# open-genome/dna

Measured on AMD Instinct MI355X. Metric: MLM sequences/sec, DNABERT-2-117M seq_len=512, at 1/2/4/8 MI355X, higher is better.
Workload: dtype bf16

## Files before the change

### dna_amd/_native.py

```python
import ctypes
import os
import re

import torch

_HERE = os.path.dirname(os.path.abspath(__file__))
LIB_PATH = os.environ.get("DNA_AMD_LIB", os.path.join(_HERE, "lib", "libdna_amd.so"))
HEADER = os.path.join(os.path.dirname(_HERE), "include", "dna_amd.h")

F32, BF16, F16 = 0, 1, 2
ACT_NONE, ACT_GELU = 0, 1

_vp, _i, _u64, _f, _sz = ctypes.c_void_p, ctypes.c_int, ctypes.c_uint64, ctypes.c_float, ctypes.c_size_t
_i64 = ctypes.c_int64

_SIGS = {
    "dna_abi_version": (_i, []),
    "dna_last_error": (ctypes.c_char_p, []),
    "dna_attn_fwd": (_i, [_vp, _vp, _vp, _i, _i, _i, _i, _i, _f, _vp, _vp, _vp]),
    "dna_attn_bwd": (_i, [_vp, _vp, _vp, _vp, _vp, _vp, _i, _i, _i, _i, _i, _f, _vp, _vp, _vp]),
    "dna_attn_bwd_ex": (_i, [_vp, _vp, _vp, _vp, _vp, _vp, _i, _i, _i, _i, _i, _f, _vp, _vp, _vp, _vp]),
    "dna_attn_dbias_part_rows": (_i, [_i, _i]),
    "dna_flash_lse_rows": (_i, [_i]),
    "dna_flash_fwd": (_i, [_vp, _i, _vp, _i, _i, _i64, _i64, _i64, _i, _i, _i, _i, _i, _f, _vp, _vp, _vp]),
    "dna_flash_bwd": (_i, [_vp, _i, _vp, _i, _i, _i64, _i64, _i64, _vp, _vp, _vp, _i, _i, _i, _i, _i,
                           _f, _vp, _vp, _vp]),
    "dna_colsum_f32": (_i, [_vp, _i, _i, _vp, _i, _vp]),
    "dna_colsum_bf16_workspace": (_sz, [_i, _i]),
    "dna_colsum_bf16": (_i, [_vp, _i, _i, _vp, _i, _vp, _sz, _vp]),
    "dna_flip_rows": (_i, [_vp, _i, _i, _sz, _vp, _vp]),
    "dna_causal_conv1d_fwd": (_i, [_vp, _sz, _i, _vp, _vp, _i, _i, _i, _i, _i, _vp, _vp]),
    "dna_causal_conv1d_part_rows": (_sz, [_i, _i]),
    "dna_causal_conv1d_bwd": (_i, [_vp, _sz, _i, _vp, _vp, _vp, _i, _i, _i, _i, _i, _vp, _sz, _vp, _vp]),
    "dna_hyena_shortconv_fwd": (_i, [_vp, _i, _vp, _vp, _i, _i, _i, _i, _i, _vp, _vp, _vp]),
    "dna_hyena_shortconv_part_elems": (_sz, [_i, _i, _i, _i, _i]),
    "dna_hyena_shortconv_bwd": (_i, [_vp, _i, _vp, _vp, _i, _i, _i, _i, _i, _vp, _vp, _vp, _vp, _vp]),
    "dna_hyena_gate_out_fwd": (_i, [_vp, _vp, _i, _i, _i, _i, _sz, _vp, _vp]),
    "dna_hyena_gate_out_bwd": (_i, [_vp, _vp, _vp, _i, _i, _i, _i, _sz, _vp, _vp, _vp]),
    "dna_hyena_modulate_t_fwd": (_i, [_vp, _i, _vp, _vp, _f, _i, _i, _i, _vp, _vp]),
    "dna_hyena_modulate_t_bwd": (_i, [_vp, _vp, _vp, _f, _i, _i, _i, _vp, _i, _vp]),
    "dna_hyena_filter_part_elems": (_i, [_i, _i, _i, _i]),
    "dna_hyena_filter_part_stride": (_i, [_i, _i, _i]),
    "dna_hyena_filter_fwd": (_i, [_vp, _vp, _vp, _vp, _vp, _i, _vp, _vp, _vp, _vp, _f, _i, _i, _i, _i,
                                  _vp, _vp]),
    "dna_hyena_filter_bwd": (_i, [_vp, _vp, _vp, _vp, _vp, _i, _vp, _vp, _vp, _vp, _f, _i, _i, _i, _i,
                                  _vp, _vp, _vp, _vp]),
    "dna_hyena_filter_finish": (_i, [_vp, _i, _i, _i, _vp, _vp]),
    "dna_ln_fwd": (_i, [_vp, _i, _vp, _i, _f, _u64, _u64, _vp, _vp, _vp, _i, _i, _f, _vp, _vp,
                        _vp, _vp, _vp]),
    "dna_ln_bwd_workspace": (_sz, [_i, _i]),
    "dna_ln_bwd": (_i, [_vp, _vp, _vp, _i, _vp, _i, _f, _u64, _u64, _vp, _vp, _vp, _vp, _i, _i,
                        _vp, _vp, _vp, _vp, _vp, _vp, _sz, _vp]),
    "dna_ln_bwd_from_y": (_i, [_vp, _vp, _vp, _i, _f, _u64, _u64, _vp, _vp, _vp, _i, _i, _vp,
                               _vp, _vp, _vp, _vp, _vp, _sz, _vp]),
# ... 124 lines not shown
```

### dna_amd/csrc/attention.hip

```cpp
#include <stdlib.h>

#include <algorithm>
#include <type_traits>

#include "common.h"

namespace dna {
namespace attn {

constexpr int D = 64;
constexpr int BQ = 128;
constexpr int BK = 64;
constexpr float LOG2E = 1.4426950408889634f;
constexpr float LN2 = 0.6931471805599453f;
constexpr float PAD_BIAS = -10000.0f;

typedef __attribute__((address_space(3))) bf16x4 lds_bf16x4;
typedef __attribute__((ext_vector_type(4))) short s16x4;

__device__ __forceinline__ int swz_key(int r) {
  const int k = (r >> 1) & 7;
  return ((k & 1) << 2) | (k & 2) | ((k >> 2) & 1);
}
__device__ __forceinline__ int swz(int r, int c) {
// ... 1264 lines not shown
__device__ __forceinline__ float sum32(float x) {
  x += dppf<0xB1>(x);
  x += dppf<0x4E>(x);
  x += dppf<0x141>(x);
  x += dppf<0x140>(x);
  return x + __shfl_xor(x, 16, 64);
}

__device__ __forceinline__ void mfma_acc(f32x16& acc, const bf16x8& a, const bf16x8& b) {
  asm volatile("s_nop 1\n\tv_mfma_f32_32x32x16_bf16 %0, %1, %2, %0" : "+a"(acc) : "v"(a), "v"(b));
}
__device__ __forceinline__ void acc_fence(f32x16& x, f32x16& y) {
  asm volatile("s_nop 7\n\ts_nop 7\n\ts_nop 7" : "+a"(x), "+a"(y));
}

template <int KB>
constexpr size_t bwd3_red_off() {
  constexpr size_t a = (size_t)128 * KB * D * 2 + 4 * 32 * D * 2 + (size_t)128 * KB * 32 * 2 + 2 * 4 * 32 * 4;
  return a > 65536 ? a : 65536;
}
constexpr int CS_LD = 36;
template <int KB>
constexpr bool bwd3_stage_alias() { return (size_t)4 * 32 * D * 2 + (size_t)128 * KB * 32 * 2 >= 4 * 64 * CS_LD * 4; }
template <int KB>
constexpr size_t bwd3_lds() {
  return bwd3_red_off<KB>() + 2 * 1024 * 4 + (size_t)128 * KB * 2 * 4 +
         (bwd3_stage_alias<KB>() ? 0 : 4 * 64 * CS_LD * 4);
}

#ifndef DNA_BWD3_STAMP
#define DNA_BWD3_STAMP 0
#endif
#if DNA_BWD3_STAMP
__device__ unsigned long long g_bwd3_stamps[4][16][6];
#define BWD3_STAMP(t, k)                                                              \
  do {                                                                                \
    const unsigned long long ts_ = __builtin_amdgcn_s_memtime();                     \
    if (blockIdx.x == 0 && lane == 0 && (t) < 16) g_bwd3_stamps[wave][(t)][(k)] = ts_; \
  } while (0)
#else
#define BWD3_STAMP(t, k) do {} while (0)
#endif
template <int KB, int V>
__global__ __launch_bounds__(256, 1) void bwd3_bf16_kernel(
    const bf16* __restrict__ qkv, const bf16* __restrict__ out, const bf16* __restrict__ dout,
    const float* __restrict__ lse, const uint8_t* __restrict__ key_valid,
    const float* __restrict__ slopes, int H, float c, float scale, bf16* __restrict__ dqkv,
    float* __restrict__ dbias_part) {
  constexpr bool DB = V & 1;
  constexpr bool DBL = DB, DBE = DB;
  constexpr bool PIPE_SB = (V & 2) != 0;
  constexpr int S = 128 * KB;
  constexpr int KPW = 32 * KB;
  constexpr int NS = S / 32;
  constexpr int KS2 = S / 32;
  extern __shared__ __attribute__((aligned(16))) char smem[];
  bf16* Kimg = reinterpret_cast<bf16*>(smem);
  bf16* Qimg = Kimg + S * D;
  bf16* Oimg = Qimg + 2 * 32 * D;
  bf16* dST = Oimg + 2 * 32 * D;
  float* rc = reinterpret_cast<float*>(dST + S * 32);
  float* red = reinterpret_cast<float*>(smem + bwd3_red_off<KB>());

  const int bh = blockIdx.x, h = bh % H, b = bh / H;
  const int tid = threadIdx.x, lane = tid & 63;
  const int wave = __builtin_amdgcn_readfirstlane(tid >> 6);
  const int kl = lane & 31, hh = lane >> 5;
  const int g16 = lane >> 4, i16 = lane & 15;
  const int ld = 3 * H * D;
  const bf16* base = qkv + (size_t)b * S * ld;
  const size_t obase = (size_t)b * S * (H * D) + h * D;
  const float slope2 = slopes[h] * LOG2E;
  const float invc = 1.f / c;
  const float sl_t = slope2 * invc;
  const float* lse_bh = lse + ((size_t)b * H + h) * S;

  {
    constexpr int NCH = S * 8 / 256;
    bf16x8 kt[NCH];
#pragma unroll
    for (int i = 0; i < NCH; ++i) {
      const int cc = tid + 256 * i;
      kt[i] = *reinterpret_cast<const bf16x8*>(base + (size_t)(cc >> 3) * ld + H * D + h * D + (cc & 7) * 8);
    }
#pragma unroll
    for (int i = 0; i < NCH; ++i) {
      const int cc = tid + 256 * i;
      *reinterpret_cast<bf16x8*>(Kimg + swz(cc >> 3, (cc & 7) * 8)) = kt[i];
    }
  }
  bf16x8 vf[KB][4];
  unsigned padm = 0;
#pragma unroll
  for (int kb = 0; kb < KB; ++kb) {
    const int kj = wave * KPW + 32 * kb + kl;
#pragma unroll
    for (int s = 0; s < 4; ++s)
      vf[kb][s] = *reinterpret_cast<const bf16x8*>(base + (size_t)kj * ld + 2 * H * D + h * D + 16 * s + 8 * hh);
    if (key_valid && !key_valid[(size_t)b * S + kj]) padm |= 1u << kb;
  }

  struct SRegs { bf16x8 q, o, d; float l; };
  auto load_slice = [&](int t, SRegs& x, int tid_t) {
    const int sr = tid_t >> 3, sc = tid_t & 7;
    const int q = 32 * t + sr;
    x.q = *reinterpret_cast<const bf16x8*>(base + (size_t)q * ld + h * D + sc * 8);
    x.o = *reinterpret_cast<const bf16x8*>(out + obase + (size_t)q * (H * D) + sc * 8);
    x.d = *reinterpret_cast<const bf16x8*>(dout + obase + (size_t)q * (H * D) + sc * 8);
// ... 9 lines not shown
    dl += dppf<0xB1>(dl);
    dl += dppf<0x4E>(dl);
    dl += dppf<0x141>(dl);
    if (sc == 0) {
      const float l2 = x.l * LOG2E, sq = slope2 * (float)(32 * t + sr);
      float* R = rc + buf * 128 + sr;
      R[0] = (-l2 - sq) * invc;
      R[32] = (-l2 + sq) * invc;
      R[64] = -l2 * invc;
      R[96] = -dl;
    }
  };

  f32x16 dk[KB][2], dv[KB][2];
  float* sigl = red + 2 * 1024;
  if (DBL)
    for (int i = tid; i < 2 * S; i += 256) sigl[i] = 0.f;
#pragma unroll
  for (int kb = 0; kb < KB; ++kb) {
#pragma unroll
    for (int i = 0; i < 16; ++i) { dk[kb][0][i] = dk[kb][1][i] = dv[kb][0][i] = dv[kb][1][i] = 0.f; }
  }
  const int dth = wave & 1, kh2 = wave >> 1;
  const bf16* Kw = Kimg + wave * KPW * D;
  bf16* dSTw = dST + wave * KPW * 32;
  const bf16* Kh = Kimg + kh2 * (S / 2) * D;
  const bf16* dSTh = dST + kh2 * (S / 2) * 32;
  {
    SRegs x;
    load_slice(0, x, tid);
    store_slice(0, 0, x, tid);
  }
  __syncthreads();

  for (int t = 0; t < NS; ++t) {
    BWD3_STAMP(t, 0);
    const int buf = t & 1;
    int tid_t = tid;
    asm volatile("" : "+v"(tid_t));
    const int kl_t = tid_t & 31;
    unsigned padm_t = padm;
    asm volatile("" : "+v"(padm_t));
    SRegs nx;
    const bf16* Q = Qimg + buf * 32 * D;
    const bf16* O = Oimg + buf * 32 * D;
    const float* RC = rc + buf * 128;
    const int qb = 32 * t;
    bf16x8 pbp[2], sbp[2];
    const int tq = 4 * (g16 >> 1) + (i16 >> 2);
    auto tr_pair = [&](const bf16* img, int j) {
      const int qrow = 16 * (j >> 1) + tq;
      const int dcol = 32 * (j & 1) + 16 * (g16 & 1) + 4 * (i16 & 3);
      return cat(tr_read(img + swz(qrow, dcol)), tr_read(img + swz(qrow + 8, dcol)));
    };
    bf16x8 qfr[4], ofr[4];
#pragma unroll
    for (int s = 0; s < 4; ++s) {
      qfr[s] = *reinterpret_cast<const bf16x8*>(Q + swz(kl, 16 * s + 8 * hh));
      ofr[s] = *reinterpret_cast<const bf16x8*>(O + swz(kl, 16 * s + 8 * hh));
    }
#pragma unroll
    for (int kb = 0; kb <= KB; ++kb) {
      __builtin_amdgcn_sched_barrier(0);
      if (kb == KB && t + 1 < NS) load_slice(t + 1, nx, tid_t);
      const int kbase = wave * KPW + 32 * kb;
      const bool after = qb > kbase, before = qb < kbase;
// ... 98 lines not shown
      };
#pragma unroll
      for (int ks = 0; ks < PF; ++ks) rd(ks, ra[ks], rb[ks]);
#pragma unroll
      for (int ks = 0; ks < KS2; ++ks) {
        dq = mfma(ra[ks % PF], rb[ks % PF], dq);
        if (ks + PF < KS2) rd(ks + PF, ra[ks % PF], rb[ks % PF]);
      }
    }
    float* rw = red + dth * 1024;
#pragma unroll
    for (int g2 = 0; g2 < 2; ++g2) {
      const int g = 2 * (1 - kh2) + g2;
      *reinterpret_cast<f32x4*>(rw + g * 256 + lane * 4) = f32x4{dq[4 * g], dq[4 * g + 1], dq[4 * g + 2], dq[4 * g + 3]};
    }
    BWD3_STAMP(t, 3);
    if (t + 1 < NS) store_slice(buf ^ 1, t + 1, nx, tid_t);
    __syncthreads();
    BWD3_STAMP(t, 4);
    {
      bf16* row = dqkv + ((size_t)b * S + qb + kl) * ld + h * D + 32 * dth;
#pragma unroll
      for (int g2 = 0; g2 < 2; ++g2) {
        const int g = 2 * kh2 + g2;
        const f32x4 v = *reinterpret_cast<const f32x4*>(rw + g * 256 + lane * 4);
        bf16x4 o;
#pragma unroll
        for (int e = 0; e < 4; ++e) o[e] = (bf16)((dq[4 * g + e] + v[e]) * scale);
        *reinterpret_cast<bf16x4*>(row + 8 * g + 4 * hh) = o;
      }
    }
    BWD3_STAMP(t, 5);
  }

#pragma unroll
  for (int kb = 0; kb < KB; ++kb)
#pragma unroll
    for (int dt = 0; dt < 2; ++dt) acc_fence(dk[kb][dt], dv[kb][dt]);
#pragma unroll
  for (int kb = 0; kb < KB; ++kb) {
    bf16* row = dqkv + ((size_t)b * S + wave * KPW + 32 * kb + kl) * ld + h * D;
#pragma unroll
    for (int dt = 0; dt < 2; ++dt)
#pragma unroll
      for (int g = 0; g < 4; ++g) {
        bf16x4 vk, vv;
#pragma unroll
        for (int e = 0; e < 4; ++e) {
          vk[e] = (bf16)(dk[kb][dt][4 * g + e] * scale);
          vv[e] = (bf16)dv[kb][dt][4 * g + e];
        }
        *reinterpret_cast<bf16x4*>(row + H * D + 32 * dt + 8 * g + 4 * hh) = vk;
        *reinterpret_cast<bf16x4*>(row + 2 * H * D + 32 * dt + 8 * g + 4 * hh) = vv;
      }
  }
  if (DBE) {
#pragma unroll
    for (int kb = 0; kb < KB; ++kb)
#pragma unroll
      for (int dt = 0; dt < 2; ++dt) asm volatile("" : "+a"(dk[kb][dt]), "+a"(dv[kb][dt]));
    __syncthreads();
    int lane_e = lane;
    asm volatile("" : "+v"(lane_e));
    const int kl_e = lane_e & 31, hh_e = lane_e >> 5;
    float* cs = red;
    float* st = (bwd3_stage_alias<KB>() ? reinterpret_cast<float*>(Qimg)
                                        : red + 2 * 1024 + 2 * S) + wave * 64 * CS_LD;
    auto rowsum = [&](float* dst) {
      f32x4 a = *reinterpret_cast<const f32x4*>(st + lane_e * CS_LD);
#pragma unroll
      for (int k = 4; k < 32; k += 4) {
        const f32x4 v = *reinterpret_cast<const f32x4*>(st + lane_e * CS_LD + k);
        a[0] += v[0]; a[1] += v[1]; a[2] += v[2]; a[3] += v[3];
      }
      *dst = (a[0] + a[1]) + (a[2] + a[3]);
    };
    {
      float sgm[KB];
#pragma unroll
      for (int kb = 0; kb < KB; ++kb) {
        const int key = wave * KPW + 32 * kb + kl_e;
        sgm[kb] = sigl[key] + sigl[S + key];
      }
#pragma unroll
      for (int cc = 0; cc < 4; ++cc) {
        float a8[8] = {0.f, 0.f, 0.f, 0.f, 0.f, 0.f, 0.f, 0.f};
#pragma unroll
        for (int kb = 0; kb < KB; ++kb) {
          const int r = wave * KPW + 32 * kb + kl_e;
          const bf16x8 v = *reinterpret_cast<const bf16x8*>(Kimg + r * D + (((4 * hh_e + cc) ^ swz_key(r)) << 3));
#pragma unroll
          for (int e = 0; e < 8; ++e) a8[e] = fmaf((float)v[e], sgm[kb], a8[e]);
        }
#pragma unroll
        for (int e = 0; e < 8; ++e) st[(32 * hh_e + 8 * cc + e) * CS_LD + kl_e] = a8[e] * scale;
      }
      rowsum(cs + (wave * 3) * 64 + lane_e);
    }
#pragma unroll
    for (int ts = 0; ts < 2; ++ts) {
#pragma unroll
      for (int dt = 0; dt < 2; ++dt)
#pragma unroll
        for (int r = 0; r < 16; ++r) {
          float sum = 0.f;
#pragma unroll
          for (int kb = 0; kb < KB; ++kb) sum += ts == 0 ? dk[kb][dt][r] : dv[kb][dt][r];
          st[(32 * dt + aoff(r) + 4 * hh_e) * CS_LD + kl_e] = ts == 0 ? sum * scale : sum;
        }
      rowsum(cs + (wave * 3 + 1 + ts) * 64 + lane_e);
    }
    __syncthreads();
    for (int i = tid; i < KB * 192; i += 256) {
      const int j = i / 192, ts = (i >> 6) % 3, d = i & 63;
      float sum = 0.f;
#pragma unroll
      for (int w = 0; w < 4 / KB; ++w) sum += cs[((j * 4 / KB + w) * 3 + ts) * 64 + d];
      dbias_part[((size_t)b * KB + j) * ld + ts * H * D + h * D + d] = sum;
    }
  }
}

constexpr int F32_TILE = 64;

__device__ __forceinline__ float bias_nat(float slope, int i, int j, const uint8_t* kv, size_t off) {
  float bb = -slope * fabsf((float)(i - j));
  if (kv && !kv[off + j]) bb += PAD_BIAS;
  return bb;
}

__global__ __launch_bounds__(64) void fwd_f32_kernel(const float* __restrict__ qkv,
                                                      const uint8_t* __restrict__ kv,
                                                      const float* __restrict__ slopes, int S,
                                                      int H, float scale, float* __restrict__ out,
                                                      float* __restrict__ lse) {
  __shared__ float Kt[F32_TILE][D + 1], Vt[F32_TILE][D + 1];
  const int h = blockIdx.y, b = blockIdx.z, t = threadIdx.x;
  const int qi = blockIdx.x * F32_TILE + t;
  const int ld = 3 * H * D;
  const float* base = qkv + (size_t)b * S * ld;
  const float slope = slopes[h];
  float q[D], o[D];
  const int qr = min(qi, S - 1);
  for (int d = 0; d < D; ++d) { q[d] = base[(size_t)qr * ld + h * D + d]; o[d] = 0.f; }
  float m = -INFINITY, l = 0.f;
  for (int k0 = 0; k0 < S; k0 += F32_TILE) {
    __syncthreads();
    for (int idx = t; idx < F32_TILE * D; idx += 64) {
      int r = idx / D, d = idx % D, j = min(k0 + r, S - 1);
      Kt[r][d] = base[(size_t)j * ld + H * D + h * D + d];
      Vt[r][d] = base[(size_t)j * ld + 2 * H * D + h * D + d];
    }
    __syncthreads();
// ... 188 lines not shown
  }
  DNA_LAUNCH_CHECK("dna_attn_fwd");
  return DNA_OK;
}

template <int KB>
static void launch_bwd3(const void* qkv, const void* out, const void* dout, const float* lse,
                        const uint8_t* key_valid, const float* slopes, int batch, int heads, float c,
                        float scale, void* dqkv, float* dbias_part, hipStream_t s) {
  static const bool attr = [] {
    const void* ks[] = {(const void*)bwd3_bf16_kernel<KB, 0>, (const void*)bwd3_bf16_kernel<KB, 1>,
                        (const void*)bwd3_bf16_kernel<KB, 2>, (const void*)bwd3_bf16_kernel<KB, 3>};
    for (const void* k : ks)
      (void)hipFuncSetAttribute(k, hipFuncAttributeMaxDynamicSharedMemorySize, (int)bwd3_lds<KB>());
    return true;
  }();
  (void)attr;
  static const bool sb = getenv("DNA_ATTN_BWD3_SB") && atoi(getenv("DNA_ATTN_BWD3_SB")) == 1;
  const dim3 grid(batch * heads);
  const size_t lds = bwd3_lds<KB>();
  auto args = [&](auto kern, float* part) {
    hipLaunchKernelGGL(kern, grid, dim3(256), lds, s, (const bf16*)qkv, (const bf16*)out,
                       (const bf16*)dout, lse, key_valid, slopes, heads, c, scale, (bf16*)dqkv, part);
  };
  if (!dbias_part) {
    if (sb) args(bwd3_bf16_kernel<KB, 2>, nullptr);
    else args(bwd3_bf16_kernel<KB, 0>, nullptr);
  } else {
    if (sb) args(bwd3_bf16_kernel<KB, 3>, dbias_part);
    else args(bwd3_bf16_kernel<KB, 1>, dbias_part);
  }
}

extern "C" int dna_attn_bwd_ex(const void* qkv, const void* out, const void* dout,
                               const float* lse, const uint8_t* key_valid, const float* slopes,
                               int batch, int seqlen, int heads, int head_dim, int dtype,
                               float softmax_scale, void* dqkv, float* delta_ws, float* dbias_part,
                               void* stream) {
  int st = check_common(qkv, slopes, batch, seqlen, heads, head_dim, dtype, "dna_attn_bwd");
  if (st) return st;
  DNA_CHECK_ARG(out && dout && lse && dqkv && delta_ws, "dna_attn_bwd: null pointer");
  hipStream_t s = as_stream(stream);
  const int rows = batch * seqlen;
  const int nd = (rows * heads + 255) / 256;
  static const int bwd_ver = getenv("DNA_ATTN_BWD") ? atoi(getenv("DNA_ATTN_BWD")) : 3;
  const bool bwd_v1 = bwd_ver == 1;
  if (dtype == DNA_BF16 && bwd_ver == 3 && (seqlen == 128 || seqlen == 256 || seqlen == 512)) {
    const float c = softmax_scale * LOG2E;
    if (seqlen == 512)
      launch_bwd3<4>(qkv, out, dout, lse, key_valid, slopes, batch, heads, c, softmax_scale, dqkv, dbias_part, s);
    else if (seqlen == 256)
      launch_bwd3<2>(qkv, out, dout, lse, key_valid, slopes, batch, heads, c, softmax_scale, dqkv, dbias_part, s);
    else
      launch_bwd3<1>(qkv, out, dout, lse, key_valid, slopes, batch, heads, c, softmax_scale, dqkv, dbias_part, s);
  } else if (dtype == DNA_BF16 && !bwd_v1) {
    static const int nw_env = getenv("DNA_ATTN_BWD_NW") ? atoi(getenv("DNA_ATTN_BWD_NW")) : 8;
    const bool w8 = nw_env == 8 && seqlen % 256 == 0;
    const size_t red = (w8 ? 8 : 4) * 32 * 64 * sizeof(float);
    const size_t dq_lds = std::max(FWD_LDS, dbias_part ? red : (size_t)0);
    const size_t kv_lds = std::max(DKDV2_LDS, dbias_part ? red : (size_t)0);
    if (w8) {
      hipLaunchKernelGGL((dq2_bf16_kernel<8>), dim3((seqlen / 256) * heads * batch), dim3(512),
                         dq_lds, s, (const bf16*)qkv, (const bf16*)out, (const bf16*)dout, lse,
                         delta_ws, key_valid, slopes, seqlen, heads, softmax_scale * LOG2E,
                         softmax_scale, (bf16*)dqkv, dbias_part);
      hipLaunchKernelGGL((dkdv2_bf16_kernel<8>), dim3((seqlen / 256) * heads * batch), dim3(512),
                         kv_lds, s, (const bf16*)qkv, (const bf16*)dout, lse, delta_ws, key_valid,
                         slopes, seqlen, heads, softmax_scale * LOG2E, softmax_scale, (bf16*)dqkv,
                         dbias_part);
    } else {
      hipLaunchKernelGGL((dq2_bf16_kernel<4>), dim3(((seqlen + BQ - 1) / BQ) * heads * batch),
                         dim3(256), dq_lds, s, (const bf16*)qkv, (const bf16*)out,
                         (const bf16*)dout, lse, delta_ws, key_valid, slopes, seqlen, heads,
                         softmax_scale * LOG2E, softmax_scale, (bf16*)dqkv, dbias_part);
      hipLaunchKernelGGL((dkdv2_bf16_kernel<4>), dim3(((seqlen + BKW - 1) / BKW) * heads * batch),
                         dim3(256), kv_lds, s, (const bf16*)qkv, (const bf16*)dout, lse, delta_ws,
                         key_valid, slopes, seqlen, heads, softmax_scale * LOG2E, softmax_scale,
                         (bf16*)dqkv, dbias_part);
    }
  } else if (dtype == DNA_BF16) {
    hipLaunchKernelGGL(dq_bf16_kernel, dim3(((seqlen + BQ - 1) / BQ) * heads * batch), dim3(256),
                       FWD_LDS, s, (const bf16*)qkv, (const bf16*)out, (const bf16*)dout, lse,
                       delta_ws, key_valid, slopes, seqlen, heads, softmax_scale * LOG2E,
                       softmax_scale, (bf16*)dqkv, dbias_part);
    hipLaunchKernelGGL(dkdv_bf16_kernel, dim3(((seqlen + BKW - 1) / BKW) * heads * batch), dim3(256),
                       DKDV_LDS, s, (const bf16*)qkv, (const bf16*)dout, lse, delta_ws, key_valid,
                       slopes, seqlen, heads, softmax_scale * LOG2E, softmax_scale, (bf16*)dqkv,
                       dbias_part);
  } else {
    DNA_CHECK_ARG(!dbias_part, "dna_attn_bwd_ex: fused bias-gradient partials need the bf16 path");
    hipLaunchKernelGGL(delta_kernel<float>, dim3(nd), dim3(256), 0, s, (const float*)out,
                       (const float*)dout, rows, heads, seqlen, delta_ws);
    dim3 grid((seqlen + F32_TILE - 1) / F32_TILE, heads, batch);
    hipLaunchKernelGGL(dq_f32_kernel, grid, dim3(64), 0, s, (const float*)qkv, (const float*)dout,
                       lse, delta_ws, key_valid, slopes, seqlen, heads, softmax_scale,
                       (float*)dqkv);
    hipLaunchKernelGGL(dkdv_f32_kernel, grid, dim3(64), 0, s, (const float*)qkv,
                       (const float*)dout, lse, delta_ws, key_valid, slopes, seqlen, heads,
                       softmax_scale, (float*)dqkv);
  }
  DNA_LAUNCH_CHECK("dna_attn_bwd");
  return DNA_OK;
}

extern "C" int dna_attn_bwd(const void* qkv, const void* out, const void* dout, const float* lse,
                            const uint8_t* key_valid, const float* slopes, int batch, int seqlen,
                            int heads, int head_dim, int dtype, float softmax_scale, void* dqkv,
                            float* delta_ws, void* stream) {
  return dna_attn_bwd_ex(qkv, out, dout, lse, key_valid, slopes, batch, seqlen, heads, head_dim,
                         dtype, softmax_scale, dqkv, delta_ws, nullptr, stream);
}

#if DNA_BWD3_STAMP
extern "C" int dna_attn_debug_stamps(unsigned long long* out) {
  return hipMemcpyFromSymbol(out, HIP_SYMBOL(g_bwd3_stamps), sizeof(g_bwd3_stamps)) == hipSuccess ? 0 : 1;
}
#endif

extern "C" int dna_attn_dbias_part_rows(int batch, int seqlen) {
  return batch * ((seqlen + BQ - 1) / BQ);
}
```

### include/dna_amd.h

```cpp
#ifndef DNA_AMD_H
#define DNA_AMD_H

#include <stddef.h>
#include <stdint.h>

#ifdef __cplusplus
extern "C" {
#endif

#define DNA_AMD_ABI_VERSION 1

enum dna_status {
  DNA_OK = 0,
  DNA_ERR_INVALID = 1,
  DNA_ERR_HIP = 2,
  DNA_ERR_UNSUPPORTED = 3,
  DNA_ERR_IO = 4,
  DNA_ERR_NOMEM = 5
};

enum dna_dtype { DNA_F32 = 0, DNA_BF16 = 1, DNA_F16 = 2 };
enum dna_act { DNA_ACT_NONE = 0, DNA_ACT_GELU = 1 };

int dna_abi_version(void);
const char* dna_last_error(void);

int dna_attn_fwd(const void* qkv, const uint8_t* key_valid, const float* slopes, int batch,
                 int seqlen, int heads, int head_dim, int dtype, float softmax_scale, void* out,
                 float* lse, void* stream);

int dna_flash_lse_rows(int seqlen);
int dna_flash_fwd(const void* qkv, int dtype, const void* bias, int bias_dtype, int bias_type,
                  long long bias_sb, long long bias_sh, long long bias_sq, int batch, int seqlen,
                  int heads, int head_dim, int causal, float softmax_scale, void* out, float* lse,
                  void* stream);
int dna_flash_bwd(const void* qkv, int dtype, const void* bias, int bias_dtype, int bias_type,
                  long long bias_sb, long long bias_sh, long long bias_sq, const void* out,
                  const void* dout, const float* lse, int batch, int seqlen, int heads,
                  int head_dim, int causal, float softmax_scale, float* delta, void* dqkv,
                  void* stream);

int dna_attn_bwd(const void* qkv, const void* out, const void* dout, const float* lse,
                 const uint8_t* key_valid, const float* slopes, int batch, int seqlen, int heads,
                 int head_dim, int dtype, float softmax_scale, void* dqkv, float* delta_ws,
                 void* stream);
int dna_attn_bwd_ex(const void* qkv, const void* out, const void* dout, const float* lse,
                    const uint8_t* key_valid, const float* slopes, int batch, int seqlen, int heads,
                    int head_dim, int dtype, float softmax_scale, void* dqkv, float* delta_ws,
                    float* dbias_part, void* stream);
int dna_attn_dbias_part_rows(int batch, int seqlen);

int dna_ln_fwd(const void* x, int x_dtype, const float* bias, int act, float p_drop,
               uint64_t seed, uint64_t offset, const float* residual, const float* gamma,
               const float* beta, int rows, int cols, float eps, float* y, void* y_bf16,
               float* mean, float* rstd, void* stream);

size_t dna_ln_bwd_workspace(int rows, int cols);
int dna_ln_bwd(const float* dy, const void* dy_bf16, const void* x, int x_dtype,
               const float* bias, int act, float p_drop, uint64_t seed, uint64_t offset,
               const float* residual, const float* gamma, const float* mean, const float* rstd,
               int rows, int cols, float* dresidual, void* dx, float* dgamma, float* dbeta,
               float* dbias, void* workspace, size_t workspace_bytes, void* stream);
int dna_ln_bwd_from_y(const float* dy, const void* dy_bf16, const float* y, int x_dtype,
                      float p_drop, uint64_t seed, uint64_t offset, const float* gamma,
                      const float* beta, const float* rstd, int rows, int cols, float* dresidual,
                      void* dx, float* dgamma, float* dbeta, float* dbias, void* workspace,
                      size_t workspace_bytes, void* stream);
int dna_ln_bwd_from_y_acc(const float* dy, const void* dy_bf16, const float* y, int x_dtype,
                          float p_drop, uint64_t seed, uint64_t offset, const float* gamma,
                          const float* beta, const float* rstd, int rows, int cols,
                          float* dresidual, void* dx, float* dgamma, float* dbeta, float* dbias,
                          void* workspace, size_t workspace_bytes, void* stream);

int dna_add_ln_fwd(const void* x, int x_dtype, const float* residual, const float* gamma,
                   const float* beta, int rows, int cols, float eps, int rms, float* sum, float* y,
                   void* y_bf16, float* mean, float* rstd, void* stream);
int dna_add_ln_bwd(const float* dy, const void* dy_bf16, const float* dsum, const void* x,
                   int x_dtype, const float* residual, const float* gamma, const float* mean,
                   const float* rstd, int rows, int cols, int rms, float* dresidual, void* dx,
                   float* dgamma, float* dbeta, void* workspace, size_t workspace_bytes,
                   void* stream);

// ... 198 lines not shown
```

Measured before the change: 2425.

## Add 8-wave fused attention backward kernel and default to it at seq 512

Adds a new 512-thread attention backward kernel in which each of eight waves owns 32*KB keys, so a 512-token head is handled with KB=2 instead of the old 4-wave KB=4 layout. It uses raw LDS addressing with ds_read_tr transpose loads, a cross-wave dQ reduction through LDS, and stages dK/dV stores through the dead Q/O images. It becomes the default for seqlen 512, and a new dna_attn_bwd_var entry point selects 4 or 8 waves explicitly. The aim is more waves per CU and fewer accumulator registers per wave, traded against extra LDS reduction traffic and more barrier synchronisation.

```diff
diff --git a/dna_amd/_native.py b/dna_amd/_native.py
--- a/dna_amd/_native.py
+++ b/dna_amd/_native.py
@@ -20,6 +20,7 @@
     "dna_attn_fwd": (_i, [_vp, _vp, _vp, _i, _i, _i, _i, _i, _f, _vp, _vp, _vp]),
     "dna_attn_bwd": (_i, [_vp, _vp, _vp, _vp, _vp, _vp, _i, _i, _i, _i, _i, _f, _vp, _vp, _vp]),
     "dna_attn_bwd_ex": (_i, [_vp, _vp, _vp, _vp, _vp, _vp, _i, _i, _i, _i, _i, _f, _vp, _vp, _vp, _vp]),
+    "dna_attn_bwd_var": (_i, [_vp, _vp, _vp, _vp, _vp, _vp, _i, _i, _i, _i, _i, _f, _vp, _vp, _vp, _i, _vp]),
     "dna_attn_dbias_part_rows": (_i, [_i, _i]),
     "dna_flash_lse_rows": (_i, [_i]),
     "dna_flash_fwd": (_i, [_vp, _i, _vp, _i, _i, _i64, _i64, _i64, _i, _i, _i, _i, _i, _f, _vp, _vp, _vp]),
diff --git a/dna_amd/csrc/attention.hip b/dna_amd/csrc/attention.hip
--- a/dna_amd/csrc/attention.hip
+++ b/dna_amd/csrc/attention.hip
@@ -1320,11 +1320,11 @@
 #define DNA_BWD3_STAMP 0
 #endif
 #if DNA_BWD3_STAMP
-__device__ unsigned long long g_bwd3_stamps[4][16][6];
+__device__ unsigned long long g_bwd3_stamps[8][17][6];
 #define BWD3_STAMP(t, k)                                                              \
   do {                                                                                \
     const unsigned long long ts_ = __builtin_amdgcn_s_memtime();                     \
-    if (blockIdx.x == 0 && lane == 0 && (t) < 16) g_bwd3_stamps[wave][(t)][(k)] = ts_; \
+    if (blockIdx.x == 0 && lane == 0 && (t) < 17) g_bwd3_stamps[wave][(t)][(k)] = ts_; \
   } while (0)
 #else
 #define BWD3_STAMP(t, k) do {} while (0)
@@ -1362,6 +1362,7 @@
   const float invc = 1.f / c;
   const float sl_t = slope2 * invc;
   const float* lse_bh = lse + ((size_t)b * H + h) * S;
+  BWD3_STAMP(16, 0);
 
   {
     constexpr int NCH = S * 8 / 256;
@@ -1437,6 +1438,7 @@
     store_slice(0, 0, x, tid);
   }
   __syncthreads();
+  BWD3_STAMP(16, 1);
 
   for (int t = 0; t < NS; ++t) {
     BWD3_STAMP(t, 0);
@@ -1601,6 +1603,7 @@
     }
     BWD3_STAMP(t, 5);
   }
+  BWD3_STAMP(16, 2);
 
 #pragma unroll
   for (int kb = 0; kb < KB; ++kb)
@@ -1623,6 +1626,7 @@
         *reinterpret_cast<bf16x4*>(row + 2 * H * D + 32 * dt + 8 * g + 4 * hh) = vv;
       }
   }
+  BWD3_STAMP(16, 3);
   if (DBE) {
 #pragma unroll
     for (int kb = 0; kb < KB; ++kb)
@@ -1688,6 +1692,419 @@
       dbias_part[((size_t)b * KB + j) * ld + ts * H * D + h * D + d] = sum;
     }
   }
+  BWD3_STAMP(16, 4);
+}
+
+typedef __attribute__((address_space(3))) char lds_byte;
+__device__ __forceinline__ unsigned lds_addr(const void* p) { return (unsigned)(size_t)(lds_byte*)p; }
+template <typename T>
+__device__ __forceinline__ T lds_ld(unsigned a) {
+  return *(const __attribute__((address_space(3))) T*)(size_t)a;
+}
+template <typename T>
+__device__ __forceinline__ void lds_st(unsigned a, T v) {
+  *(__attribute__((address_space(3))) T*)(size_t)a = v;
+}
+__device__ __forceinline__ bf16x4 tr_read_a(unsigned a) {
+  s16x4 v = __builtin_amdgcn_ds_read_tr16_b64_v4i16((__attribute__((address_space(3))) s16x4*)(size_t)a);
+  return __builtin_bit_cast(bf16x4, v);
+}
+
+template <int KB>
+constexpr size_t bwd8_red_off() {
+  return (size_t)256 * KB * D * 2 + 4 * 32 * D * 2 + (size_t)256 * KB * 32 * 2 + 2 * 4 * 32 * 4;
+}
+constexpr size_t BWD8_RED = 2 * 4 * 3 * 256 * 4;
+template <int KB>
+constexpr size_t bwd8_sig_off() {
+  constexpr size_t a = bwd8_red_off<KB>() + BWD8_RED;
+  constexpr size_t st_end = (size_t)256 * KB * D * 2 + 4 * 64 * CS_LD * 4;
+  return a > st_end ? a : st_end;
+}
+template <int KB>
+constexpr size_t bwd8_lds() { return bwd8_sig_off<KB>() + (size_t)256 * KB * 2 * 4 + 4 * 3 * 64 * 4; }
+
+#if DNA_BWD3_STAMP
+#define BWD8_STAMP(t, k) BWD3_STAMP(t, k)
+#else
+#define BWD8_STAMP(t, k) do {} while (0)
+#endif
+template <int KB, bool DB>
+__global__ __launch_bounds__(512, 2) void bwd3w8_bf16_kernel(
+    const bf16* __restrict__ qkv, const bf16* __restrict__ out, const bf16* __restrict__ dout,
+    const float* __restrict__ lse, const uint8_t* __restrict__ key_valid,
+    const float* __restrict__ slopes, int H, float c, float scale, bf16* __restrict__ dqkv,
+    float* __restrict__ dbias_part) {
+  static_assert(KB == 1 || KB == 2, "8 waves x 32*KB keys: S = 256 or 512");
+  static_assert(bwd8_lds<KB>() <= 160 * 1024, "LDS map");
+  constexpr int S = 256 * KB;
+  constexpr int KPW = 32 * KB;
+  constexpr int NS = S / 32;
+  constexpr int KS2 = S / 64;
+  extern __shared__ __attribute__((aligned(16))) char smem[];
+  bf16* Kimg = reinterpret_cast<bf16*>(smem);
+  bf16* Qimg = Kimg + S * D;
+  bf16* Oimg = Qimg + 2 * 32 * D;
+  bf16* dST = Oimg + 2 * 32 * D;
+  float* rc = reinterpret_cast<float*>(dST + S * 32);
+  float* red = reinterpret_cast<float*>(smem + bwd8_red_off<KB>());
+  float* sigl = reinterpret_cast<float*>(smem + bwd8_sig_off<KB>());
+
+  const int bh = blockIdx.x, h = bh % H, b = bh / H;
+  const int tid = threadIdx.x, lane = tid & 63;
+  const int wave = __builtin_amdgcn_readfirstlane(tid >> 6);
+  const int kl = lane & 31, hh = lane >> 5;
+  const int g16 = lane >> 4, i16 = lane & 15;
+  const int ld = 3 * H * D;
+  const bf16* base = qkv + (size_t)b * S * ld;
+  const size_t obase = (size_t)b * S * (H * D) + h * D;
+  const float slope2 = slopes[h] * LOG2E;
+  const float invc = 1.f / c;
+  const float sl_t = slope2 * invc;
+  const float* lse_bh = lse + ((size_t)b * H + h) * S;
+  BWD8_STAMP(16, 0);
+
+  {
+    constexpr int NCH = S * 8 / 512;
+    bf16x8 kt[NCH];
+#pragma unroll
+    for (int i = 0; i < NCH; ++i) {
+      const int cc = tid + 512 * i;
+      kt[i] = *reinterpret_cast<const bf16x8*>(base + (size_t)(cc >> 3) * ld + H * D + h * D + (cc & 7) * 8);
+    }
+#pragma unroll
+    for (int i = 0; i < NCH; ++i) {
+      const int cc = tid + 512 * i;
+      *reinterpret_cast<bf16x8*>(Kimg + swz(cc >> 3, (cc & 7) * 8)) = kt[i];
+    }
+  }
+  bf16x8 vf[4];
+  const bf16* vbase = base + 2 * H * D + h * D;
+#pragma unroll
+  for (int s = 0; s < 4; ++s)
+    vf[s] = *reinterpret_cast<const bf16x8*>(vbase + (size_t)(wave * KPW + kl) * ld + 8 * hh + 16 * s);
+  unsigned padm = 0;
+#pragma unroll
+  for (int kb = 0; kb < KB; ++kb)
+    if (key_valid && !key_valid[(size_t)b * S + wave * KPW + 32 * kb + kl]) padm |= 1u << kb;
+
+  const bool stager = wave < 4;
+  struct SRegs { bf16x8 q, o, d; float l; };
+  auto load_slice = [&](int t, SRegs& x, int tid_t) {
+    const int sr = tid_t >> 3, sc = tid_t & 7;
+    const int q = 32 * t + sr;
+    x.q = *reinterpret_cast<const bf16x8*>(base + (size_t)q * ld + h * D + sc * 8);
+    x.o = *reinterpret_cast<const bf16x8*>(out + obase + (size_t)q * (H * D) + sc * 8);
+    x.d = *reinterpret_cast<const bf16x8*>(dout + obase + (size_t)q * (H * D) + sc * 8);
+    x.l = lse_bh[q];
+  };
+  auto store_slice = [&](int buf, int t, const SRegs& x, int tid_t) {
+    const int sr = tid_t >> 3, sc = tid_t & 7;
+    *reinterpret_cast<bf16x8*>(Qimg + buf * 32 * D + swz(sr, sc * 8)) = x.q;
+    *reinterpret_cast<bf16x8*>(Oimg + buf * 32 * D + swz(sr, sc * 8)) = x.d;
+    float dl = 0.f;
+#pragma unroll
+    for (int j = 0; j < 8; ++j) dl = fmaf((float)x.d[j], (float)x.o[j], dl);
+    dl += dppf<0xB1>(dl);
+    dl += dppf<0x4E>(dl);
+    dl += dppf<0x141>(dl);
+    if (sc == 0) {
+      const float l2 = x.l * LOG2E, sq = slope2 * (float)(32 * t + sr);
+      float* R = rc + buf * 128 + sr;
+      R[0] = (-l2 - sq) * invc;
+      R[32] = (-l2 + sq) * invc;
+      R[64] = -l2 * invc;
+      R[96] = -dl;
+    }
+  };
+
+  f32x16 dk[KB][2], dv[KB][2];
+  if (DB)
+    for (int i = tid; i < 2 * S; i += 512) sigl[i] = 0.f;
+#pragma unroll
+  for (int kb = 0; kb < KB; ++kb) {
+#pragma unroll
+    for (int i = 0; i < 16; ++i) { dk[kb][0][i] = dk[kb][1][i] = dv[kb][0][i] = dv[kb][1][i] = 0.f; }
+  }
+  const int dth = wave & 1, kq = wave >> 1;
+  const int tq0 = 4 * (g16 >> 1) + (i16 >> 2), tc0 = 16 * (g16 & 1) + 4 * (i16 & 3);
+  unsigned a_f = 2 * swz(kl, 8 * hh);
+  unsigned a_t = 2 * swz(tq0, tc0);
+  unsigned a_d = lds_addr(dST + wave * KPW * 32) + 2 * (kl * 32 + 4 * (hh ^ ((kl >> 1) & 7)));
+  unsigned a_s = lds_addr(dST + kq * (S / 4) * 32) + 2 * (tq0 * 32 + 4 * ((tc0 >> 2) ^ ((tq0 >> 1) & 7)));
+  unsigned a_g = lds_addr(sigl + hh * S + wave * KPW + kl);
+  unsigned v_off = (unsigned)(wave * KPW + kl) * (unsigned)ld + 8 * hh;
+  const unsigned s_K = lds_addr(Kimg + wave * KPW * D), s_Kq = lds_addr(Kimg + kq * (S / 4) * D);
+  const unsigned s_red = lds_addr(red + dth * (4 * 3 * 256));
+  if (stager) {
+    SRegs x;
+    load_slice(0, x, tid);
+    store_slice(0, 0, x, tid);
+  }
+  __syncthreads();
+  BWD8_STAMP(16, 1);
+
+  for (int t = 0; t < NS; ++t) {
+    BWD8_STAMP(t, 0);
+    const int buf = t & 1;
+    int tid_t = tid;
+    asm volatile("" : "+v"(tid_t));
+    unsigned padm_t = padm;
+    asm volatile("" : "+v"(padm_t));
+    SRegs nx;
+    const unsigned s_Q = lds_addr(Qimg + buf * 32 * D);
+    constexpr unsigned O_OFF = 2 * 32 * D * 2;
+    const unsigned s_rc = lds_addr(rc + buf * 128);
+    const int qb = 32 * t;
+#pragma unroll
+    for (int kb = 0; kb < KB; ++kb) {
+      __builtin_amdgcn_sched_barrier(0);
+      asm volatile("" : "+v"(a_f), "+v"(a_g), "+v"(v_off));
+      const int hh_b = (tid_t >> 5) & 1;
+      const int kbase = wave * KPW + 32 * kb;
+      const bool after = qb > kbase, before = qb < kbase;
+      const int sel = after ? 0 : (before ? 1 : 2);
+      const unsigned a_rc = s_rc + sel * 128 + 16 * hh_b, a_dl = s_rc + 3 * 128 + 16 * hh_b;
+      f32x16 sa, pa;
+#pragma unroll
+      for (int g4 = 0; g4 < 4; ++g4) {
+        const f32x4 l4 = lds_ld<f32x4>(a_rc + 32 * g4);
+#pragma unroll
+        for (int e = 0; e < 4; ++e) sa[4 * g4 + e] = l4[e];
+      }
+#pragma unroll
+      for (int g4 = 0; g4 < 4; ++g4) {
+        const f32x4 d4 = lds_ld<f32x4>(a_dl + 32 * g4);
+#pragma unroll
+        for (int e = 0; e < 4; ++e) pa[4 * g4 + e] = d4[e];
+      }
+      const unsigned a_q = a_f + s_Q, a_k = a_f + s_K;
+#pragma unroll
+      for (int s = 0; s < 4; ++s) {
+        const bf16x8 of = lds_ld<bf16x8>((a_q ^ (32 * s)) + O_OFF);
+        const bf16x8 qf = lds_ld<bf16x8>(a_q ^ (32 * s));
+        const bf16x8 kr = lds_ld<bf16x8>((a_k ^ (32 * s)) + kb * 32 * D * 2);
+        pa = mfma(of, vf[s], pa);
+        sa = mfma(qf, kr, sa);
+      }
+      if (KB > 1) {
+#pragma unroll
+        for (int s = 0; s < 4; ++s)
+          vf[s] = *reinterpret_cast<const bf16x8*>(vbase + (v_off + ((kb + 1) % KB) * 32 * ld) + 16 * s);
+      }
+      const int kl_b = tid_t & 31;
+      const float kbias = ((padm_t >> kb) & 1) ? PAD_BIAS * LOG2E : 0.f;
+      const float U = (after || before) ? fmaf(after ? slope2 : -slope2, (float)(kbase + kl_b), kbias) : kbias;
+      if (!after && !before) {
+        float lq = (float)(4 * hh_b - kl_b);
+        asm volatile("" : "+v"(lq));
+#pragma unroll
+        for (int r = 0; r < 16; ++r) sa[r] = fmaf(-sl_t, fabsf(lq + (float)aoff(r)), sa[r]);
+      }
+      const float sold = DB ? lds_ld<float>(a_g + kb * 32 * 4) : 0.f;
+      bf16x8 pb[2], sb[2];
+      float ssum = 0.f;
+#pragma unroll
+      for (int r = 0; r < 16; ++r) {
+        const float pr = ex2(fmaf(sa[r], c, U));
+        const float ds = pr * pa[r];
+        pb[r >> 3][r & 7] = (bf16)pr;
+        sb[r >> 3][r & 7] = (bf16)ds;
+        if (DB) ssum += ds;
+      }
+      if (DB) lds_st<float>(a_g + kb * 32 * 4, sold + ssum);
+      if (kb == KB - 1 && t + 1 < NS && stager) load_slice(t + 1, nx, tid_t);
+      asm volatile("" : "+v"(a_d), "+v"(a_t));
+#pragma unroll
+      for (int g = 0; g < 4; ++g) {
+        const bf16x8& src = sb[g >> 1];
+        const bf16x4 v = {src[4 * (g & 1)], src[4 * (g & 1) + 1], src[4 * (g & 1) + 2], src[4 * (g & 1) + 3]};
+        lds_st<bf16x4>((a_d ^ (16 * g)) + kb * 32 * 32 * 2, v);
+      }
+      const unsigned a_tq = a_t + s_Q;
+      auto tr_pair = [&](unsigned img_off, int j) {
+        const unsigned a0 = (a_tq ^ (64 * (j & 1))) + img_off + (j >> 1) * 16 * D * 2;
+        const unsigned a1 = (a_tq ^ (64 * (j & 1) + 16)) + img_off + (j >> 1) * 16 * D * 2 + 8 * D * 2;
+        return cat(tr_read_a(a0), tr_read_a(a1));
+      };
+      bf16x8 ao[2], aq[2];
+      ao[0] = tr_pair(O_OFF, 0); aq[0] = tr_pair(0, 0);
+      ao[1] = tr_pair(O_OFF, 1); aq[1] = tr_pair(0, 1);
+#pragma unroll
+      for (int j = 0; j < 4; ++j) {
+        mfma_acc(dv[kb][j & 1], ao[j & 1], pb[j >> 1]);
+        mfma_acc(dk[kb][j & 1], aq[j & 1], sb[j >> 1]);
+        if (j < 2) { ao[j & 1] = tr_pair(O_OFF, j + 2); aq[j & 1] = tr_pair(0, j + 2); }
+      }
+    }
+    BWD8_STAMP(t, 1);
+    __syncthreads();
+    BWD8_STAMP(t, 2);
+    f32x16 dq;
+#pragma unroll
+    for (int i = 0; i < 16; ++i) dq[i] = 0.f;
+    asm volatile("" : "+v"(a_t), "+v"(a_s));
+    {
+      const unsigned a_k0 = (a_t ^ (64 * dth)) + s_Kq;
+      constexpr int PF = KS2 < 4 ? KS2 : 4;
+      bf16x8 ra[PF], rb[PF];
+      auto rd = [&](int ks, bf16x8& a, bf16x8& bb) {
+        a = cat(tr_read_a(a_k0 + ks * 16 * D * 2), tr_read_a((a_k0 ^ 16) + ks * 16 * D * 2 + 8 * D * 2));
+        bb = cat(tr_read_a(a_s + ks * 16 * 32 * 2), tr_read_a((a_s ^ 32) + ks * 16 * 32 * 2 + 8 * 32 * 2));
+      };
+#pragma unroll
+      for (int ks = 0; ks < PF; ++ks) rd(ks, ra[ks], rb[ks]);
+#pragma unroll
+      for (int ks = 0; ks < KS2; ++ks) {
+        dq = mfma(ra[ks % PF], rb[ks % PF], dq);
+        if (ks + PF < KS2) rd(ks + PF, ra[ks % PF], rb[ks % PF]);
+      }
+    }
+    const unsigned a_red = s_red + 16 * (tid_t & 63);
+#pragma unroll
+    for (int g = 0; g < 4; ++g)
+      if (g != kq)
+        lds_st<f32x4>(a_red + (kq * 3 + (g > kq ? g - 1 : g)) * 1024,
+                      f32x4{dq[4 * g], dq[4 * g + 1], dq[4 * g + 2], dq[4 * g + 3]});
+    BWD8_STAMP(t, 3);
+    if (t + 1 < NS && stager) store_slice(buf ^ 1, t + 1, nx, tid_t);
+    __syncthreads();
+    BWD8_STAMP(t, 4);
+    {
+      bf16* row = dqkv + (size_t)b * S * ld + h * D + 32 * dth +
+                  ((unsigned)(qb + (tid_t & 31)) * (unsigned)ld + 4 * ((tid_t >> 5) & 1));
+#pragma unroll
+      for (int g = 0; g < 4; ++g)
+        if (g == kq) {
+          f32x4 p[4];
+#pragma unroll
+          for (int ks = 0; ks < 4; ++ks)
+            p[ks] = ks == g ? f32x4{dq[4 * g], dq[4 * g + 1], dq[4 * g + 2], dq[4 * g + 3]}
+                            : lds_ld<f32x4>(a_red + (ks * 3 + (g > ks ? g - 1 : g)) * 1024);
+          bf16x4 o;
+#pragma unroll
+          for (int e = 0; e < 4; ++e) o[e] = (bf16)(((p[0][e] + p[1][e]) + (p[2][e] + p[3][e])) * scale);
+          *reinterpret_cast<bf16x4*>(row + 8 * g) = o;
+        }
+    }
+    BWD8_STAMP(t, 5);
+  }
+  BWD8_STAMP(16, 2);
+
+#pragma unroll
+  for (int kb = 0; kb < KB; ++kb)
+#pragma unroll
+    for (int dt = 0; dt < 2; ++dt) acc_fence(dk[kb][dt], dv[kb][dt]);
+  static_assert(8 * 4096 <= 4 * 32 * D * 2 + S * 32 * 2, "store tiles fit the dead images");
+  {
+    const unsigned a_w = lds_addr(Qimg) + wave * 4096 + kl * 128 + ((kl & 7) << 4) + 8 * hh;
+    const int srow = lane >> 3, sch = lane & 7;
+    const unsigned a_r = lds_addr(Qimg) + wave * 4096 + srow * 128 + ((sch ^ srow) << 4);
+    bf16* grow = dqkv + ((size_t)b * S + wave * KPW + srow) * ld + h * D + 8 * sch;
+#pragma unroll
+    for (int kb = 0; kb < KB; ++kb)
+#pragma unroll
+      for (int ts = 0; ts < 2; ++ts) {
+#pragma unroll
+        for (int dt = 0; dt < 2; ++dt)
+#pragma unroll
+          for (int g = 0; g < 4; ++g) {
+            bf16x4 v;
+#pragma unroll
+            for (int e = 0; e < 4; ++e)
+              v[e] = ts == 0 ? (bf16)(dk[kb][dt][4 * g + e] * scale) : (bf16)dv[kb][dt][4 * g + e];
+            lds_st<bf16x4>(a_w ^ ((4 * dt + g) << 4), v);
+          }
+#pragma unroll
+        for (int i = 0; i < 4; ++i)
+          *reinterpret_cast<bf16x8*>(grow + (size_t)(32 * kb + 8 * i) * ld + (1 + ts) * H * D) =
+              lds_ld<bf16x8>(a_r + i * 8 * 128);
+      }
+  }
+  BWD8_STAMP(16, 3);
+  if (DB) {
+#pragma unroll
+    for (int kb = 0; kb < KB; ++kb)
+#pragma unroll
+      for (int dt = 0; dt < 2; ++dt) asm volatile("" : "+a"(dk[kb][dt]), "+a"(dv[kb][dt]));
+    __syncthreads();
+    int lane_e = lane;
+    asm volatile("" : "+v"(lane_e));
+    const int kl_e = lane_e & 31, hh_e = lane_e >> 5;
+    const int pair = wave >> 1;
+    const bool odd = (wave & 1) != 0;
+    float* cs = sigl + 2 * S;
+    float* st = reinterpret_cast<float*>(Qimg) + pair * 64 * CS_LD;
+    auto rowsum = [&](float* dst) {
+      f32x4 a = *reinterpret_cast<const f32x4*>(st + lane_e * CS_LD);
+#pragma unroll
+      for (int k = 4; k < 32; k += 4) {
+        const f32x4 v = *reinterpret_cast<const f32x4*>(st + lane_e * CS_LD + k);
+        a[0] += v[0]; a[1] += v[1]; a[2] += v[2]; a[3] += v[3];
+      }
+      *dst = (a[0] + a[1]) + (a[2] + a[3]);
+    };
+    auto dq_part = [&](bool first) {
+      float sgm[KB];
+#pragma unroll
+      for (int kb = 0; kb < KB; ++kb) {
+        const int key = wave * KPW + 32 * kb + kl_e;
+        sgm[kb] = sigl[key] + sigl[S + key];
+      }
+#pragma unroll
+      for (int cc = 0; cc < 4; ++cc) {
+        float a8[8];
+#pragma unroll
+        for (int e = 0; e < 8; ++e) a8[e] = first ? 0.f : st[(32 * hh_e + 8 * cc + e) * CS_LD + kl_e];
+#pragma unroll
+        for (int kb = 0; kb < KB; ++kb) {
+          const int r = wave * KPW + 32 * kb + kl_e;
+          const bf16x8 v = *reinterpret_cast<const bf16x8*>(Kimg + r * D + (((4 * hh_e + cc) ^ swz_key(r)) << 3));
+#pragma unroll
+          for (int e = 0; e < 8; ++e) a8[e] = fmaf((float)v[e], sgm[kb], a8[e]);
+        }
+#pragma unroll
+        for (int e = 0; e < 8; ++e) st[(32 * hh_e + 8 * cc + e) * CS_LD + kl_e] = first ? a8[e] : a8[e] * scale;
+      }
+    };
+    if (!odd) dq_part(true);
+    __syncthreads();
+    if (odd) {
+      dq_part(false);
+      rowsum(cs + (pair * 3) * 64 + lane_e);
+    }
+    __syncthreads();
+#pragma unroll
+    for (int ts = 0; ts < 2; ++ts) {
+      auto acc_part = [&](bool first) {
+#pragma unroll
+        for (int dt = 0; dt < 2; ++dt)
+#pragma unroll
+          for (int r = 0; r < 16; ++r) {
+            float* p = st + (32 * dt + aoff(r) + 4 * hh_e) * CS_LD + kl_e;
+            float sum = first ? 0.f : *p;
+#pragma unroll
+            for (int kb = 0; kb < KB; ++kb) sum += ts == 0 ? dk[kb][dt][r] : dv[kb][dt][r];
+            *p = (first || ts == 1) ? sum : sum * scale;
+          }
+      };
+      if (!odd) acc_part(true);
+      __syncthreads();
+      if (odd) {
+        acc_part(false);
+        rowsum(cs + (pair * 3 + 1 + ts) * 64 + lane_e);
+      }
+      __syncthreads();
+    }
+    for (int i = tid; i < 2 * KB * 192; i += 512) {
+      const int j = i / 192, ts = (i >> 6) % 3, d = i & 63;
+      float sum = 0.f;
+#pragma unroll
+      for (int w = 0; w < 2 / KB; ++w) sum += cs[((j * 2 / KB + w) * 3 + ts) * 64 + d];
+      dbias_part[((size_t)b * 2 * KB + j) * ld + ts * H * D + h * D + d] = sum;
+    }
+  }
+  BWD8_STAMP(16, 4);
 }
 
 constexpr int F32_TILE = 64;
@@ -1942,22 +2359,53 @@
   }
 }
 
-extern "C" int dna_attn_bwd_ex(const void* qkv, const void* out, const void* dout,
-                               const float* lse, const uint8_t* key_valid, const float* slopes,
-                               int batch, int seqlen, int heads, int head_dim, int dtype,
-                               float softmax_scale, void* dqkv, float* delta_ws, float* dbias_part,
-                               void* stream) {
+template <int KB>
+static void launch_bwd3w8(const void* qkv, const void* out, const void* dout, const float* lse,
+                          const uint8_t* key_valid, const float* slopes, int batch, int heads,
+                          float c, float scale, void* dqkv, float* dbias_part, hipStream_t s) {
+  static const bool attr = [] {
+    const void* ks[] = {(const void*)bwd3w8_bf16_kernel<KB, false>, (const void*)bwd3w8_bf16_kernel<KB, true>};
+    for (const void* k : ks)
+      (void)hipFuncSetAttribute(k, hipFuncAttributeMaxDynamicSharedMemorySize, (int)bwd8_lds<KB>());
+    return true;
+  }();
+  (void)attr;
+  const dim3 grid(batch * heads);
+  const size_t lds = bwd8_lds<KB>();
+  auto args = [&](auto kern, float* part) {
+    hipLaunchKernelGGL(kern, grid, dim3(512), lds, s, (const bf16*)qkv, (const bf16*)out,
+                       (const bf16*)dout, lse, key_valid, slopes, heads, c, scale, (bf16*)dqkv, part);
+  };
+  if (!dbias_part) args(bwd3w8_bf16_kernel<KB, false>, nullptr);
+  else args(bwd3w8_bf16_kernel<KB, true>, dbias_part);
+}
+
+static int bwd3_nw_default(int seqlen) {
+  static const int nw = getenv("DNA_ATTN_BWD3_NW") ? atoi(getenv("DNA_ATTN_BWD3_NW")) : 0;
+  return nw ? nw : (seqlen == 512 ? 8 : 4);
+}
+
+static int attn_bwd_impl(const void* qkv, const void* out, const void* dout, const float* lse,
+                         const uint8_t* key_valid, const float* slopes, int batch, int seqlen,
+                         int heads, int head_dim, int dtype, float softmax_scale, void* dqkv,
+                         float* delta_ws, float* dbias_part, int nw, void* stream) {
   int st = check_common(qkv, slopes, batch, seqlen, heads, head_dim, dtype, "dna_attn_bwd");
   if (st) return st;
   DNA_CHECK_ARG(out && dout && lse && dqkv && delta_ws, "dna_attn_bwd: null pointer");
   hipStream_t s = as_stream(stream);
   const int rows = batch * seqlen;
   const int nd = (rows * heads + 255) / 256;
-  static const int bwd_ver = getenv("DNA_ATTN_BWD") ? atoi(getenv("DNA_ATTN_BWD")) : 3;
+  static const int bwd_env = getenv("DNA_ATTN_BWD") ? atoi(getenv("DNA_ATTN_BWD")) : 3;
+  const int bwd_ver = nw ? 3 : bwd_env;
   const bool bwd_v1 = bwd_ver == 1;
   if (dtype == DNA_BF16 && bwd_ver == 3 && (seqlen == 128 || seqlen == 256 || seqlen == 512)) {
     const float c = softmax_scale * LOG2E;
-    if (seqlen == 512)
+    const bool w8 = (nw ? nw : bwd3_nw_default(seqlen)) == 8 && seqlen != 128;
+    if (w8 && seqlen == 512)
+      launch_bwd3w8<2>(qkv, out, dout, lse, key_valid, slopes, batch, heads, c, softmax_scale, dqkv, dbias_part, s);
+    else if (w8)
+      launch_bwd3w8<1>(qkv, out, dout, lse, key_valid, slopes, batch, heads, c, softmax_scale, dqkv, dbias_part, s);
+    else if (seqlen == 512)
       launch_bwd3<4>(qkv, out, dout, lse, key_valid, slopes, batch, heads, c, softmax_scale, dqkv, dbias_part, s);
     else if (seqlen == 256)
       launch_bwd3<2>(qkv, out, dout, lse, key_valid, slopes, batch, heads, c, softmax_scale, dqkv, dbias_part, s);
@@ -2013,6 +2461,29 @@
   return DNA_OK;
 }
 
+extern "C" int dna_attn_bwd_ex(const void* qkv, const void* out, const void* dout,
+                               const float* lse, const uint8_t* key_valid, const float* slopes,
+                               int batch, int seqlen, int heads, int head_dim, int dtype,
+                               float softmax_scale, void* dqkv, float* delta_ws, float* dbias_part,
+                               void* stream) {
+  return attn_bwd_impl(qkv, out, dout, lse, key_valid, slopes, batch, seqlen, heads, head_dim, dtype,
+                       softmax_scale, dqkv, delta_ws, dbias_part, 0, stream);
+}
+
+extern "C" int dna_attn_bwd_var(const void* qkv, const void* out, const void* dout,
+                                const float* lse, const uint8_t* key_valid, const float* slopes,
+                                int batch, int seqlen, int heads, int head_dim, int dtype,
+                                float softmax_scale, void* dqkv, float* delta_ws, float* dbias_part,
+                                int nw, void* stream) {
+  DNA_CHECK_ARG(nw == 4 || nw == 8, "dna_attn_bwd_var: nw %d (4 or 8)", nw);
+  if (dtype != DNA_BF16 || !(seqlen == 512 || seqlen == 256 || (nw == 4 && seqlen == 128))) {
+    set_error("dna_attn_bwd_var: no %d-wave fused backward for dtype %d, seqlen %d", nw, dtype, seqlen);
+    return DNA_ERR_UNSUPPORTED;
+  }
+  return attn_bwd_impl(qkv, out, dout, lse, key_valid, slopes, batch, seqlen, heads, head_dim, dtype,
+                       softmax_scale, dqkv, delta_ws, dbias_part, nw, stream);
+}
+
 extern "C" int dna_attn_bwd(const void* qkv, const void* out, const void* dout, const float* lse,
                             const uint8_t* key_valid, const float* slopes, int batch, int seqlen,
                             int heads, int head_dim, int dtype, float softmax_scale, void* dqkv,
diff --git a/include/dna_amd.h b/include/dna_amd.h
--- a/include/dna_amd.h
+++ b/include/dna_amd.h
@@ -48,6 +48,10 @@
                     const uint8_t* key_valid, const float* slopes, int batch, int seqlen, int heads,
                     int head_dim, int dtype, float softmax_scale, void* dqkv, float* delta_ws,
                     float* dbias_part, void* stream);
+int dna_attn_bwd_var(const void* qkv, const void* out, const void* dout, const float* lse,
+                     const uint8_t* key_valid, const float* slopes, int batch, int seqlen, int heads,
+                     int head_dim, int dtype, float softmax_scale, void* dqkv, float* delta_ws,
+                     float* dbias_part, int nw, void* stream);
 int dna_attn_dbias_part_rows(int batch, int seqlen);
 
 int dna_ln_fwd(const void* x, int x_dtype, const float* bias, int act, float p_drop,
```

Result: faster. 2466, median of 6 (+1.7%).
